# EPFL-VILAB/omnidata

Measured on AMD Instinct MI355X. Metric: images/sec (384x384) DPT-Hybrid surface-normal inference, higher is better.
Workload: dtype bf16; 1 GPU; DPT-Hybrid-384 normal, batch 32/GPU, bf16, 1xMI355X (BASELINE.json configs[1]); batch_per_gpu=32, global_batch=32, parallelism=replicas x1 (no collective in the loop), ranks_seen=1, inflight=1

## Files before the change

include/dptx.h:

```cpp
#ifndef DPTX_H_
#define DPTX_H_

#include <stddef.h>
#include <stdint.h>

#ifdef __cplusplus
extern "C" {
#endif

typedef struct dptx_engine* dptx_handle;

enum {
  DPTX_OK = 0,
  DPTX_E_INVALID = -1,
  DPTX_E_KEY = -2,
  DPTX_E_HIP = -3,
  DPTX_E_NODEVICE = -4,
  DPTX_E_ALLOC = -5
};

enum { DPTX_DTYPE_BF16 = 0, DPTX_DTYPE_FP16 = 1, DPTX_DTYPE_BF16X3 = 2,
       DPTX_DTYPE_FP16X3 = 3, DPTX_DTYPE_MIXED = 4,
       DPTX_DTYPE_FP8 = 5 };
enum { DPTX_GROUP_RESNET = 1,
// ... 165 lines not shown
int dptx_eval_normal_pixels(const float* pred, const float* target, int32_t B, int32_t H, int32_t W, double* ang, void* stream);


int dptx_op_set_planes(int64_t act_plane_elems, int64_t w_plane_elems);

int dptx_op_gemm(int32_t dtype, const void* A, const void* W, const float* bias, const void* R,
                 void* C, int32_t M, int32_t N, int32_t K, int32_t act, int32_t a_fp32,
                 int32_t c_fp32, int32_t r_fp32, void* stream);
int dptx_op_conv(int32_t dtype, const void* X, const void* Wt, const float* bias, const void* R,
                 void* Y, int32_t B, int32_t H, int32_t W, int32_t Cin, int32_t Cout,
                 int32_t ksize, int32_t stride, int32_t pad_t, int32_t pad_l, int32_t Ho,
                 int32_t Wo, int32_t a_relu, int32_t act, void* stream);
int dptx_op_conv_planes(int32_t dtype, const void* X, const void* Wt, const float* bias, const void* R, void* Y, int32_t B,
                        int32_t H, int32_t W, int32_t Cin, int32_t Cout, int32_t ksize, int32_t stride, int32_t pad_t,
                        int32_t pad_l, int32_t Ho, int32_t Wo, int32_t a_relu, int32_t act, int32_t epi2, int32_t c_hi_only,
                        int32_t r1_hi_only, void* stream);
int dptx_op_stem_conv(int32_t dtype, const float* x, const void* Wt, void* y, int32_t B, int32_t H, int32_t W,
                      void* stream);
int dptx_op_attention(int32_t dtype, const void* qkv, void* out, int32_t B, int32_t S,
                      int32_t heads, void* stream);
int dptx_op_layernorm(int32_t dtype, const float* x, const float* gamma, const float* beta,
                      void* y, int32_t M, int32_t C, float eps, void* stream);
int dptx_op_groupnorm(int32_t dtype, const void* X, const float* gamma, const float* beta,
                      const void* R, void* Y, int32_t B, int32_t HW, int32_t C, int32_t relu,
                      float eps, void* scratch_f32, void* stream);
int dptx_op_gn_relu_maxpool(int32_t dtype, const void* X, const float* gamma, const float* beta, void* Y, int32_t B,
                            int32_t H, int32_t W, int32_t C, float eps, void* scratch_f32, void* stream);
int dptx_op_cls_rows(int32_t dtype, const float* cls, const float* pos, float* X, int32_t B, int32_t S, int32_t C, void* X16,
                     float* row_stats, void* X8, float q_scale, void* stream);
int dptx_debug_set_trace(void* dev_buf);
int dptx_debug_arena_fill(dptx_handle h, int32_t byte_value);
int dptx_debug_arena_read(dptx_handle h, void* dst_host, size_t offset, size_t bytes);
int dptx_debug_arena_layout(dptx_handle h, char* dst, size_t capacity);
int dptx_debug_arena_checksums(dptx_handle h, void* out_dev, int32_t capacity, void* stream);
int dptx_debug_set_gemm_flags(int32_t flags);
int dptx_op_conv_fp8(const void* X8, const void* Wt8, const float* bias, const void* R, void* Y, void* Y8, int32_t B,
                     int32_t H, int32_t W, int32_t Cin, int32_t Cout, int32_t ksize, int32_t stride, int32_t pad_t,
                     int32_t pad_l, int32_t Ho, int32_t Wo, int32_t act, int32_t q_relu, float out_scale, void* stream);
int dptx_op_conv_groupnorm(int32_t dtype, const void* X, const void* Wt, void* Yraw, const float* gamma, const float* beta,
                           const void* R, void* Y, int32_t B, int32_t H, int32_t W, int32_t Cin, int32_t Cout,
                           int32_t ksize, int32_t stride, int32_t pad_t, int32_t pad_l, int32_t Ho, int32_t Wo,
                           int32_t relu, float eps, void* scratch_f32, void* stream);
int dptx_op_upsample2x(int32_t dtype, const void* X, void* Y, int32_t B, int32_t H, int32_t W,
                       int32_t C, void* stream);
int dptx_op_gemm_ln(int32_t dtype, const void* A, const void* W, const float* bias, void* C, int32_t M, int32_t N, int32_t K,
                    int32_t act, const float* ln_stats, const float* ln_colsum, int32_t ln_nblk, float ln_eps, void* stream);
int dptx_op_gemm_stream(int32_t dtype, const void* A, const void* W, const float* bias, void* C, float* row_stats, int32_t M,
                        int32_t N, int32_t K, void* stream);
int dptx_op_gemm_stream32(int32_t dtype, const void* A, const void* W, const float* bias, float* X, void* C16, float* row_stats,
                          int32_t M, int32_t N, int32_t K, void* stream);
int dptx_op_head_tail(int32_t dtype, const void* H0, const void* W2, const float* b2, const float* w4,
                      const float* b4, float* y, int32_t B, int32_t Hs, int32_t Ws, int32_t C,
                      int32_t relu_out, void* stream);

#ifdef __cplusplus
}
#endif
#endif
```

omnidata_amd/csrc/head.hip:

```cpp
#include <cstdlib>

#include "common.h"
#include "kernels.h"

namespace dptx {

constexpr int HT_THREADS = 576;
constexpr int HT_PR = 10, HT_PC = 34;
constexpr int HT_W_BYTES = 32 * 9 * 256;
constexpr int HT_P_BYTES = HT_PR * HT_PC * 256;
constexpr int HT_CONST_FLOATS = 32 + 3 * 32 + 4;
constexpr size_t HT_SMEM = HT_W_BYTES + HT_P_BYTES + HT_CONST_FLOATS * 4;

template <int DT>
__device__ __forceinline__ void unpack8(const u32x4_t v, float* f) {
  f[0] = T16<DT>::tof((uint16_t)(v.x & 0xffffu)); f[1] = T16<DT>::tof((uint16_t)(v.x >> 16));
  f[2] = T16<DT>::tof((uint16_t)(v.y & 0xffffu)); f[3] = T16<DT>::tof((uint16_t)(v.y >> 16));
  f[4] = T16<DT>::tof((uint16_t)(v.z & 0xffffu)); f[5] = T16<DT>::tof((uint16_t)(v.z >> 16));
  f[6] = T16<DT>::tof((uint16_t)(v.w & 0xffffu)); f[7] = T16<DT>::tof((uint16_t)(v.w >> 16));
}

template <int DT>
__device__ __forceinline__ void hblend(const u32x4_t s0, const u32x4_t s1, float lx0, float lx1, float (&t)[8]) {
  float a[8], b[8];
  unpack8<DT>(s0, a);
  unpack8<DT>(s1, b);
#pragma unroll
  for (int e = 0; e < 8; ++e) t[e] = __fmaf_rn(lx1, b[e], __fmul_rn(lx0, a[e]));
}
template <int DT, int J>
__device__ __forceinline__ u32x4_t vblend(const float (&T)[6][8], float ly0, float ly1) {
  float o[8];
#pragma unroll
  for (int e = 0; e < 8; ++e) o[e] = __fmaf_rn(ly1, T[J + 1][e], __fmul_rn(ly0, T[J][e]));
  u32x4_t r;
  r.x = T16<DT>::pack2(o[0], o[1]);
  r.y = T16<DT>::pack2(o[2], o[3]);
  r.z = T16<DT>::pack2(o[4], o[5]);
  r.w = T16<DT>::pack2(o[6], o[7]);
  return r;
}

template <int DT>
__global__ __launch_bounds__(HT_THREADS) void head_tail_kernel(const uint16_t* __restrict__ H0, const uint16_t* __restrict__ W2,
                                                               const float* __restrict__ b2, const float* __restrict__ w4,
                                                               const float* __restrict__ b4, void* __restrict__ y, int io, int B,
                                                               int Hs, int Ws, int C, int relu_out, int ntiles) {
  extern __shared__ __attribute__((aligned(16))) char smem[];
  char* Wl = smem;
  char* P = smem + HT_W_BYTES;
  float* cst = (float*)(smem + HT_W_BYTES + HT_P_BYTES);

  const int tid = threadIdx.x, lane = tid & 63, wave = tid >> 6;
  const int lr = lane & 31, lh = lane >> 5;
  const int Ho = 2 * Hs, Wo = 2 * Ws;
  const int tiles_x = Wo / 32, tiles_y = Ho / 8, tpi = tiles_x * tiles_y;
  const float ry = Ho > 1 ? (float)(Hs - 1) / (float)(Ho - 1) : 0.f;
  const float rx = Wo > 1 ? (float)(Ws - 1) / (float)(Wo - 1) : 0.f;

  {
    constexpr int NW = 32 * 9 * 16 / HT_THREADS;
    static_assert(NW * HT_THREADS == 32 * 9 * 16, "weight tensor splits evenly over the block");
    u32x4_t wv[NW];
#pragma unroll
    for (int j = 0; j < NW; ++j) {
      const int i = tid + j * HT_THREADS;
      const int n = i / 144, rem = i - n * 144;
      wv[j] = *(const u32x4_t*)(W2 + n * 1152 + (rem >> 4) * 128 + (rem & 15) * 8);
    }
#pragma unroll
    for (int j = 0; j < NW; ++j) {
      const int i = tid + j * HT_THREADS;
      const int n = i / 144, rem = i - n * 144, tap = rem >> 4, ch = rem & 15;
      *(u32x4_t*)(Wl + n * 2304 + tap * 256 + ((ch ^ (n & 15)) << 4)) = wv[j];
    }
  }
  if (tid < 32) cst[tid] = b2[tid];
  if (tid < 32 * C) cst[32 + tid] = w4[tid];
  if (tid < C) cst[128 + tid] = b4[tid];

  const int per = (ntiles + gridDim.x - 1) / gridDim.x;
  const int t_beg = blockIdx.x * per, t_end = min(t_beg + per, ntiles);

  const int wx = tid >> 4, wch = tid & 15;
  const bool col_thread = wx < HT_PC;

  u32x4_t S[6][2];
  const u32x4_t zero4 = {0u, 0u, 0u, 0u};

  auto fetch = [&](int t) {
    const int b = t / tpi, rem = t - b * tpi, ty = rem / tiles_x, tx = rem - ty * tiles_x;
    const int ox = tx * 32 - 1 + wx;
    const bool vx = col_thread && ox >= 0 && ox < Wo;
    const float sx = rx * (float)(vx ? ox : 0);
    const int x0 = (int)sx, x1 = x0 + (x0 < Ws - 1 ? 1 : 0);
    const int oyb = max(ty * 8 - 1, 0);
    const int ybase = (int)(ry * (float)oyb);
    const uint16_t* img = H0 + (long long)b * Hs * Ws * 128 + wch * 8;
#pragma unroll
    for (int j = 0; j < 6; ++j) {
      const int row = min(ybase + j, Hs - 1);
      S[j][0] = vx ? *(const u32x4_t*)(img + ((long long)row * Ws + x0) * 128) : zero4;
      S[j][1] = vx ? *(const u32x4_t*)(img + ((long long)row * Ws + x1) * 128) : zero4;
    }
  };

  if (t_beg < t_end) fetch(t_beg);
  __syncthreads();

  for (int t = t_beg; t < t_end; ++t) {
    const int b = t / tpi, rem = t - b * tpi, ty = rem / tiles_x, tx = rem - ty * tiles_x;
    const int oy0 = ty * 8, ox0 = tx * 32;

    if (col_thread) {
      const int ox = ox0 - 1 + wx;
      const bool vx = ox >= 0 && ox < Wo;
      const float sx = rx * (float)(vx ? ox : 0);
      const int x0 = (int)sx;
      const float lx1 = sx - (float)x0, lx0 = 1.f - lx1;
      const int ybase = (int)(ry * (float)max(oy0 - 1, 0));
      char* dst = P + wx * 256 + ((wch ^ (wx & 15)) << 4);
      float T[6][8];
#pragma unroll
      for (int j = 0; j < 6; ++j) hblend<DT>(S[j][0], S[j][1], lx0, lx1, T[j]);
      for (int r = 0; r < HT_PR; ++r) {
        const int oy = oy0 - 1 + r;
        u32x4_t o = zero4;
        if (vx && oy >= 0 && oy < Ho) {
          const float sy = ry * (float)oy;
          const int y0 = (int)sy;
          const float ly1 = sy - (float)y0, ly0 = 1.f - ly1;
          switch (y0 - ybase) {
            case 0: o = vblend<DT, 0>(T, ly0, ly1); break;
            case 1: o = vblend<DT, 1>(T, ly0, ly1); break;
            case 2: o = vblend<DT, 2>(T, ly0, ly1); break;
            case 3: o = vblend<DT, 3>(T, ly0, ly1); break;
            default: o = vblend<DT, 4>(T, ly0, ly1); break;
          }
        }
        *(u32x4_t*)(dst + r * (HT_PC * 256)) = o;
      }
    }
    if (t + 1 < t_end) fetch(t + 1);
    __syncthreads();

    if (wave < 8) {
      f32x16_t acc;
#pragma unroll
      for (int r = 0; r < 16; ++r) acc[r] = 0.f;
      const char* wrow = Wl + lr * 2304;
      const int wkey = lr & 15;
      constexpr int NB = 2, NBATCH = 8 / NB * 9;
      u32x4_t wf[2][NB], pf[2][NB];
      auto read_batch = [&](int bi, u32x4_t (&w)[NB], u32x4_t (&q)[NB]) {
        const int tap = bi / (8 / NB), cb0 = (bi % (8 / NB)) * NB;
        const int ky = tap / 3, kx = tap - ky * 3;
        const int xc = lr + kx;
        const char* prow = P + ((wave + ky) * HT_PC + xc) * 256;
        const int pkey = xc & 15;
#pragma unroll
        for (int i = 0; i < NB; ++i) {
          const int chunk = 2 * (cb0 + i) + lh;
          w[i] = *(const u32x4_t*)(wrow + tap * 256 + ((chunk ^ wkey) << 4));
          q[i] = *(const u32x4_t*)(prow + ((chunk ^ pkey) << 4));
        }
      };
      read_batch(0, wf[0], pf[0]);
#pragma unroll
      for (int bi = 0; bi < NBATCH; ++bi) {
        if (bi + 1 < NBATCH) read_batch(bi + 1, wf[(bi + 1) & 1], pf[(bi + 1) & 1]);
        __builtin_amdgcn_sched_barrier(0);
#pragma unroll
        for (int i = 0; i < NB; ++i) acc = T16<DT>::mfma32(wf[bi & 1][i], pf[bi & 1][i], acc);
        __builtin_amdgcn_sched_barrier(0);
      }
      float h[16];
#pragma unroll
      for (int q = 0; q < 4; ++q) {
        const float4 bb = *(const float4*)(cst + 8 * q + 4 * lh);
        h[4 * q + 0] = fmaxf(acc[4 * q + 0] + bb.x, 0.f);
        h[4 * q + 1] = fmaxf(acc[4 * q + 1] + bb.y, 0.f);
        h[4 * q + 2] = fmaxf(acc[4 * q + 2] + bb.z, 0.f);
        h[4 * q + 3] = fmaxf(acc[4 * q + 3] + bb.w, 0.f);
      }
      const int oy = oy0 + wave;
      for (int c = 0; c < C; ++c) {
        float s = 0.f;
#pragma unroll
        for (int q = 0; q < 4; ++q) {
          const float4 ww = *(const float4*)(cst + 32 + c * 32 + 8 * q + 4 * lh);
          s += ww.x * h[4 * q + 0] + ww.y * h[4 * q + 1] + ww.z * h[4 * q + 2] + ww.w * h[4 * q + 3];
        }
        s += __shfl_xor(s, 32);
        s += cst[128 + c];
        if (relu_out) s = fmaxf(s, 0.f);
        if ((c & 1) == lh) io_store(y, (((long long)b * C + c) * Ho + oy) * Wo + ox0 + lr, s, io);
      }
    }
    __syncthreads();
  }
}

constexpr int HX_THREADS = 640;
constexpr int HX_WPL = 9 * 32 * 64;
constexpr int HX_PPL = HT_PR * HT_PC * 64;
constexpr int HX_STAGE = 2 * HX_WPL + 2 * HX_PPL;
constexpr size_t HX_SMEM = 2 * HX_STAGE;
static_assert(HX_SMEM <= 160 * 1024, "one block per CU");

template <int DT>
__device__ __forceinline__ void hblend2(const u32x4_t (&s0)[2], const u32x4_t (&s1)[2], float lx0, float lx1, float (&t)[8]) {
  float a[8], b[8];
  unpack8x<DT, 2>(s0[0], s0[1], a);
  unpack8x<DT, 2>(s1[0], s1[1], b);
#pragma unroll
  for (int e = 0; e < 8; ++e) t[e] = __fmaf_rn(lx1, b[e], __fmul_rn(lx0, a[e]));
}

template <int DT>
__global__ __launch_bounds__(HX_THREADS) void head_tail_x3_kernel(const uint16_t* __restrict__ H0, const uint16_t* __restrict__ W2,
                                                                  const float* __restrict__ b2, const float* __restrict__ w4,
                                                                  const float* __restrict__ b4, void* __restrict__ y, int io, int B,
                                                                  int Hs, int Ws, int C, int relu_out, int ntiles, long long plane,
                                                                  long long wplane) {
#if defined(__HIP_DEVICE_COMPILE__)
  extern __shared__ __attribute__((aligned(16))) char smem[];

  const int tid = threadIdx.x, lane = tid & 63;
  const int wave = __builtin_amdgcn_readfirstlane(tid >> 6);
  const int lr = lane & 31, lh = lane >> 5;
  const int Ho = 2 * Hs, Wo = 2 * Ws;
  const int tiles_x = Wo / 32, tiles_y = Ho / 8, tpi = tiles_x * tiles_y;
  const float ry = Ho > 1 ? (float)(Hs - 1) / (float)(Ho - 1) : 0.f;
  const float rx = Wo > 1 ? (float)(Ws - 1) / (float)(Wo - 1) : 0.f;

  const int per = (ntiles + gridDim.x - 1) / gridDim.x;
  const int t_beg = blockIdx.x * per, t_end = min(t_beg + per, ntiles);
  const int G = (t_end - t_beg) * 4;
  if (G <= 0) return;

  if (wave == 5) {
    const __amdgpu_buffer_rsrc_t rsrcW = __builtin_amdgcn_make_buffer_rsrc(const_cast<uint16_t*>(W2), 0, (int)((wplane + 32 * 1152) * 2), 0x00020000);
#pragma unroll 1
    for (int g = 0; g < G; ++g) {
      const int quarter = g & 3;
      char* Wl = smem + (g & 1) * HX_STAGE;
#pragma unroll 6
      for (int q = 0; q < 36; ++q) {
        const int pl = q / 18, r = 16 * (q % 18) + (lane >> 2);
        const int tap = r >> 5, n = r & 31;
        const int sch = (lane & 3) ^ ((n >> 2) & 3);
        const unsigned off = (unsigned)(((long long)pl * wplane + n * 1152 + tap * 128 + quarter * 32 + sch * 8) * 2);
        __builtin_amdgcn_raw_ptr_buffer_load_lds(rsrcW, (__attribute__((address_space(3))) void*)(Wl + q * 1024), 16, off, 0, 0, 0);
// ... 108 lines not shown
      }
    };
    read_ks(0, 0, wf[0], pf[0]);
#pragma unroll
    for (int ks = 0; ks < 18; ++ks) {
      if (ks + 1 < 18) read_ks((ks + 1) >> 1, (ks + 1) & 1, wf[(ks + 1) & 1], pf[(ks + 1) & 1]);
      __builtin_amdgcn_sched_barrier(0);
      acc[0] = T16<DT>::mfma32(wf[ks & 1][0], pf[ks & 1][0][1], acc[0]);
      acc[1] = T16<DT>::mfma32(wf[ks & 1][0], pf[ks & 1][1][1], acc[1]);
      acc[0] = T16<DT>::mfma32(wf[ks & 1][1], pf[ks & 1][0][0], acc[0]);
      acc[1] = T16<DT>::mfma32(wf[ks & 1][1], pf[ks & 1][1][0], acc[1]);
      acc[0] = T16<DT>::mfma32(wf[ks & 1][0], pf[ks & 1][0][0], acc[0]);
      acc[1] = T16<DT>::mfma32(wf[ks & 1][0], pf[ks & 1][1][0], acc[1]);
      __builtin_amdgcn_sched_barrier(0);
    }
    if (quarter == 3) {
      const int b = t / tpi, rem = t - b * tpi, ty = rem / tiles_x, tx = rem - ty * tiles_x;
      const int oy0 = ty * 8, ox0 = tx * 32;
#pragma unroll
      for (int i = 0; i < 2; ++i) {
        float h[16];
#pragma unroll
        for (int q = 0; q < 4; ++q) {
          const float4 bb = *(const float4*)(b2 + 8 * q + 4 * lh);
          h[4 * q + 0] = fmaxf(acc[i][4 * q + 0] + bb.x, 0.f);
          h[4 * q + 1] = fmaxf(acc[i][4 * q + 1] + bb.y, 0.f);
          h[4 * q + 2] = fmaxf(acc[i][4 * q + 2] + bb.z, 0.f);
          h[4 * q + 3] = fmaxf(acc[i][4 * q + 3] + bb.w, 0.f);
        }
        const int oy = oy0 + 2 * mw + i;
        for (int c = 0; c < C; ++c) {
          float sacc = 0.f;
#pragma unroll
          for (int q = 0; q < 4; ++q) {
            const float4 ww = *(const float4*)(w4 + c * 32 + 8 * q + 4 * lh);
            sacc += ww.x * h[4 * q + 0] + ww.y * h[4 * q + 1] + ww.z * h[4 * q + 2] + ww.w * h[4 * q + 3];
          }
          sacc += __shfl_xor(sacc, 32);
          sacc += b4[c];
          if (relu_out) sacc = fmaxf(sacc, 0.f);
          if ((c & 1) == lh) io_store(y, (((long long)b * C + c) * Ho + oy) * Wo + ox0 + lr, sacc, io);
        }
      }
    }
    if (g + 1 < G) {
      asm volatile("s_waitcnt lgkmcnt(0)" ::: "memory");
      asm volatile("s_barrier" ::: "memory");
    }
  }
#endif
}

hipError_t launch_head_tail(int mode, const void* H0, const void* W2, const float* b2, const float* w4, const float* b4,
                            void* y, int io, int B, int Hs, int Ws, int C, int relu_out, hipStream_t stream, Planes pl) {
  if (C < 1 || C > 3 || (2 * Hs) % 8 != 0 || (2 * Ws) % 32 != 0) return hipErrorInvalidValue;
  const int ntiles = B * ((2 * Hs) / 8) * ((2 * Ws) / 32);
  static int cus = 0;
  if (cus == 0) {
    int dev = 0;
    hipDeviceProp_t prop;
    if (hipGetDevice(&dev) == hipSuccess && hipGetDeviceProperties(&prop, dev) == hipSuccess) cus = prop.multiProcessorCount;
    if (cus <= 0) cus = 256;
  }
  const int grid = ntiles < cus ? ntiles : cus;
  if (mode_is_x3(mode)) {
    if (mode != MODE_FP16X3 || pl.act == 0 || pl.w == 0 || (pl.w + 32 * 1152) * 2 >= (1ll << 31)) return hipErrorInvalidValue;
    auto k = head_tail_x3_kernel<DT_FP16>;
    ensure_dyn_smem((const void*)k, HX_SMEM);
    const int grid2 = grid;
    hipLaunchKernelGGL(k, dim3(grid2), dim3(HX_THREADS), HX_SMEM, stream, (const uint16_t*)H0, (const uint16_t*)W2, b2, w4, b4, y, io, B,
                       Hs, Ws, C, relu_out, ntiles, pl.act, pl.w);
    return hipGetLastError();
  }
  if (mode == MODE_BF16) {
    auto k = head_tail_kernel<DT_BF16>;
    ensure_dyn_smem((const void*)k, HT_SMEM);
    hipLaunchKernelGGL(k, dim3(grid), dim3(HT_THREADS), HT_SMEM, stream, (const uint16_t*)H0, (const uint16_t*)W2, b2, w4, b4, y, io, B,
                       Hs, Ws, C, relu_out, ntiles);
  } else {
    auto k = head_tail_kernel<DT_FP16>;
    ensure_dyn_smem((const void*)k, HT_SMEM);
    hipLaunchKernelGGL(k, dim3(grid), dim3(HT_THREADS), HT_SMEM, stream, (const uint16_t*)H0, (const uint16_t*)W2, b2, w4, b4, y, io, B,
                       Hs, Ws, C, relu_out, ntiles);
  }
  return hipGetLastError();
}

}
```

omnidata_amd/csrc/kernels.h:

```cpp
#pragma once
#include <hip/hip_runtime.h>
#include <stdint.h>

#include "common.h"

namespace dptx {

void ensure_dyn_smem(const void* kernel, size_t bytes);

struct GemmParams {
  const void* A;
  const void* W;
  void* C;
  const float* bias;
  const void* R1;
  const void* R2;
  int M, N, K;
  int ldw;
  int a_rpi, Wout, Hin, Win, Cin, a_pix_stride;
  long long a_img_stride, a_off;
  long long a_bytes;
  int ksz, stride, pad_t, pad_l;
  int c_rpi, c_img_rows, c_row_off, ldc;
  int r2_bcast;
// ... 25 lines not shown
  long long* trace;
  int debug_flags;
  float a_rpi_rcp, wout_rcp;
};

void gemm_params_dense(GemmParams& p, int M, int N, int K);
void gemm_params_conv(GemmParams& p, int B, int Hin, int Win, int Cin, int Cout, int ksz, int stride, int pad_t, int pad_l,
                      int Hout, int Wout, int a_elem_bytes);
hipError_t launch_gemm(int dtype, const GemmParams& p, hipStream_t stream);
void gemm_set_trace(long long* dev_buf);
void gemm_set_debug_flags(int flags);
bool conv1x1_stream_eligible(int mode, const GemmParams& p);
bool conv1x1_stream_adopted(const GemmParams& p);
hipError_t launch_conv1x1_stream(int mode, const GemmParams& p, hipStream_t stream);
void gemm_set_cu_share(float share);

hipError_t launch_attention(int mode, const void* qkv, void* out, int B, int S, int heads, Planes pl, hipStream_t stream);

hipError_t launch_layernorm(int mode, const float* x, const float* gamma, const float* beta, void* y,
                            int M, int C, float eps, Planes pl, hipStream_t stream);

struct GnParams {
  const void* X; void* Y;
  const float* gamma; const float* beta;
  float* partial;
  const void* R;
  const float* r_gamma; const float* r_beta; const float* r_partial;
  int B, HW, C, relu;
  float eps;
  int nrec;
};
int gn_chunks(int HW, int C);
hipError_t launch_gn_stats(int mode, const void* X, float* partial, int B, int HW, int C, Planes pl, hipStream_t stream);
hipError_t launch_gn_apply(int mode, const GnParams& p, Planes pl, hipStream_t stream);
hipError_t launch_gn_relu_maxpool(int mode, const void* X, void* Y, const float* gamma, const float* beta,
                                  const float* partial, int B, int H, int W, int C, float eps, Planes pl, hipStream_t stream);

hipError_t launch_stem_conv(int mode, const void* x, int io, const void* Wt, void* y, int B, int H, int W, Planes pl,
                            hipStream_t stream);

hipError_t launch_upsample2x(int mode, const void* X, void* Y, int B, int H, int W, int C, Planes pl, hipStream_t stream,
                             void* Y8 = nullptr, float q_scale = 1.0f, bool out_hi_only = false);
hipError_t launch_amax(int mode, const void* X, size_t n, int relu, unsigned* amax_bits, hipStream_t stream);

hipError_t launch_nonfinite_scan(int mode, const void* X, size_t n, unsigned* flag, hipStream_t stream);

hipError_t launch_checksum(const void* p, size_t bytes, unsigned long long* out, hipStream_t stream);
hipError_t launch_spin(long long ticks_100mhz, hipStream_t stream);

hipError_t launch_head_out(int mode, const void* X, const float* w, const float* b, void* y, int io, int B, int HW,
                           int Cout, int relu, Planes pl, hipStream_t stream);

hipError_t launch_head_tail(int mode, const void* H0, const void* W2, const float* b2, const float* w4, const float* b4,
                            void* y, int io, int B, int Hs, int Ws, int C, int relu_out, hipStream_t stream, Planes pl = Planes{0, 0});
hipError_t launch_pos_resize(const float* src, float* dst, int g_old, int gh, int gw, int C, hipStream_t stream);
hipError_t launch_cls_rows(int mode, const float* cls, const float* pos, float* X, int B, int S, int C, void* X16, float* stats,
                           hipStream_t stream, void* X8 = nullptr, float q_scale = 1.0f);

hipError_t launch_readout_cls(int mode, const float* x, long long x_stride, const void* W, int ldw, int w_off,
                              const float* bias, float* out, int B, int N, int K, Planes pl, hipStream_t stream, int x16 = 0);
hipError_t launch_cast_f32(int mode, const float* src, void* dst, size_t n, Planes pl, hipStream_t stream);

hipError_t launch_patchify16(int mode, const void* x, int io, void* P, int B, int H, int W, Planes pl, hipStream_t stream);
hipError_t launch_depth_to_space(int mode, const void* G, void* Y, int B, int h, int w, int k, int C, Planes pl, hipStream_t stream);

hipError_t launch_to_f32(int mode, const void* src, float* dst, size_t n, Planes pl, hipStream_t stream);

}
```

omnidata_amd/csrc/ops.hip:

```cpp
#include <hip/hip_runtime.h>

#include "../../include/dptx.h"
#include "kernels.h"

using namespace dptx;

extern "C" {

static int rc(hipError_t r) { return r == hipSuccess ? DPTX_OK : DPTX_E_HIP; }

static Planes g_op_planes{0, 0};
int dptx_op_set_planes(int64_t act_plane_elems, int64_t w_plane_elems) {
  g_op_planes.act = act_plane_elems;
  g_op_planes.w = w_plane_elems;
  return DPTX_OK;
}

int dptx_op_gemm(int32_t dtype, const void* A, const void* W, const float* bias, const void* R, void* C, int32_t M, int32_t N,
                 int32_t K, int32_t act, int32_t a_fp32, int32_t c_fp32, int32_t r_fp32, void* stream) {
  GemmParams p;
  gemm_params_dense(p, M, N, K);
  p.A = A; p.W = W; p.C = C; p.bias = bias; p.R1 = R; p.act = act; p.a_fp32 = a_fp32; p.c_fp32 = c_fp32; p.r1_fp32 = r_fp32;
  p.planes = g_op_planes;
  return rc(launch_gemm(dtype, p, (hipStream_t)stream));
}

int dptx_op_gemm_ln(int32_t dtype, const void* A, const void* W, const float* bias, void* C, int32_t M, int32_t N, int32_t K,
                    int32_t act, const float* ln_stats, const float* ln_colsum, int32_t ln_nblk, float ln_eps, void* stream) {
  GemmParams p;
  gemm_params_dense(p, M, N, K);
  p.A = A; p.W = W; p.C = C; p.bias = bias; p.act = act; p.planes = g_op_planes;
  p.ln_stats = ln_stats; p.ln_colsum = ln_colsum; p.ln_nblk = ln_nblk; p.ln_eps = ln_eps; p.ln_inv_dim = 1.0f / (float)K;
  return rc(launch_gemm(dtype, p, (hipStream_t)stream));
}

int dptx_op_gemm_stream(int32_t dtype, const void* A, const void* W, const float* bias, void* C, float* row_stats, int32_t M,
                        int32_t N, int32_t K, void* stream) {
  GemmParams p;
  gemm_params_dense(p, M, N, K);
  p.A = A; p.W = W; p.C = C; p.R1 = C; p.bias = bias; p.planes = g_op_planes;
  p.row_stats = row_stats; p.stats_nblk = 8;
  return rc(launch_gemm(dtype, p, (hipStream_t)stream));
}

int dptx_op_gemm_stream32(int32_t dtype, const void* A, const void* W, const float* bias, float* X, void* C16, float* row_stats,
                          int32_t M, int32_t N, int32_t K, void* stream) {
  GemmParams p;
  gemm_params_dense(p, M, N, K);
  p.A = A; p.W = W; p.C = X; p.c_fp32 = 1; p.R1 = X; p.r1_fp32 = 1; p.C16 = C16; p.bias = bias; p.planes = g_op_planes;
  p.row_stats = row_stats; p.stats_nblk = 8;
  return rc(launch_gemm(dtype, p, (hipStream_t)stream));
}

int dptx_op_head_tail(int32_t dtype, const void* H0, const void* W2, const float* b2, const float* w4, const float* b4, float* y,
                      int32_t B, int32_t Hs, int32_t Ws, int32_t C, int32_t relu_out, void* stream) {
  return rc(launch_head_tail(dtype, H0, W2, b2, w4, b4, y, DPTX_IO_FP32, B, Hs, Ws, C, relu_out, (hipStream_t)stream, g_op_planes));
}

int dptx_op_conv(int32_t dtype, const void* X, const void* Wt, const float* bias, const void* R, void* Y, int32_t B, int32_t H,
                 int32_t W, int32_t Cin, int32_t Cout, int32_t ksize, int32_t stride, int32_t pad_t, int32_t pad_l, int32_t Ho,
                 int32_t Wo, int32_t a_relu, int32_t act, void* stream) {
  GemmParams p;
  gemm_params_conv(p, B, H, W, Cin, Cout, ksize, stride, pad_t, pad_l, Ho, Wo, 2);
  p.A = X; p.W = Wt; p.C = Y; p.bias = bias; p.R1 = R; p.act = act; p.a_relu = a_relu; p.planes = g_op_planes;
  return rc(launch_gemm(dtype, p, (hipStream_t)stream));
}

int dptx_op_conv_planes(int32_t dtype, const void* X, const void* Wt, const float* bias, const void* R, void* Y, int32_t B, int32_t H,
                        int32_t W, int32_t Cin, int32_t Cout, int32_t ksize, int32_t stride, int32_t pad_t, int32_t pad_l, int32_t Ho,
                        int32_t Wo, int32_t a_relu, int32_t act, int32_t epi2, int32_t c_hi_only, int32_t r1_hi_only, void* stream) {
  GemmParams p;
  gemm_params_conv(p, B, H, W, Cin, Cout, ksize, stride, pad_t, pad_l, Ho, Wo, 2);
  p.A = X; p.W = Wt; p.C = Y; p.bias = bias; p.R1 = R; p.act = act; p.a_relu = a_relu; p.planes = g_op_planes;
  p.epi2 = epi2 & 1; p.a_hi_only = (epi2 >> 1) & 1; p.c_hi_only = c_hi_only; p.r1_hi_only = r1_hi_only;
  return rc(launch_gemm(dtype, p, (hipStream_t)stream));
}

int dptx_op_stem_conv(int32_t dtype, const float* x, const void* Wt, void* y, int32_t B, int32_t H, int32_t W, void* stream) {
  return rc(launch_stem_conv(dtype, x, DPTX_IO_FP32, Wt, y, B, H, W, g_op_planes, (hipStream_t)stream));
}

int dptx_op_attention(int32_t dtype, const void* qkv, void* out, int32_t B, int32_t S, int32_t heads, void* stream) {
  return rc(launch_attention(dtype, qkv, out, B, S, heads, g_op_planes, (hipStream_t)stream));
}

int dptx_op_layernorm(int32_t dtype, const float* x, const float* gamma, const float* beta, void* y, int32_t M, int32_t C,
                      float eps, void* stream) {
  return rc(launch_layernorm(dtype, x, gamma, beta, y, M, C, eps, g_op_planes, (hipStream_t)stream));
}

int dptx_op_groupnorm(int32_t dtype, const void* X, const float* gamma, const float* beta, const void* R, void* Y, int32_t B,
                      int32_t HW, int32_t C, int32_t relu, float eps, void* scratch_f32, void* stream) {
  if (scratch_f32 == nullptr) return DPTX_E_INVALID;
  hipError_t r = launch_gn_stats(dtype, X, (float*)scratch_f32, B, HW, C, g_op_planes, (hipStream_t)stream);
  if (r != hipSuccess) return DPTX_E_HIP;
  GnParams g{};
  g.X = X; g.Y = Y; g.gamma = gamma; g.beta = beta; g.partial = (float*)scratch_f32; g.R = R;
  g.B = B; g.HW = HW; g.C = C; g.relu = relu; g.eps = eps;
  return rc(launch_gn_apply(dtype, g, g_op_planes, (hipStream_t)stream));
}

int dptx_op_gn_relu_maxpool(int32_t dtype, const void* X, const float* gamma, const float* beta, void* Y, int32_t B, int32_t H,
                            int32_t W, int32_t C, float eps, void* scratch_f32, void* stream) {
  if (scratch_f32 == nullptr) return DPTX_E_INVALID;
  hipError_t r = launch_gn_stats(dtype, X, (float*)scratch_f32, B, H * W, C, g_op_planes, (hipStream_t)stream);
  if (r != hipSuccess) return DPTX_E_HIP;
  return rc(launch_gn_relu_maxpool(dtype, X, Y, gamma, beta, (const float*)scratch_f32, B, H, W, C, eps, g_op_planes, (hipStream_t)stream));
}

// ... 47 lines not shown
```

omnidata_amd/engine.py:

```python
from __future__ import annotations

import ctypes as C
import os
from typing import Dict, Optional, Tuple

import numpy as np
import torch

_HERE = os.path.dirname(os.path.abspath(__file__))
LIB_PATH = os.environ.get("DPTX_LIB") or os.path.join(_HERE, "libdptx.so")

DTYPES = {"bf16": 0, "fp16": 1, "bf16x3": 2, "fp16x3": 3, "mixed": 4, "fp8": 5}
TWO_PLANE_DTYPES = frozenset(("bf16x3", "fp16x3", "mixed", "fp8"))
GROUPS = {"resnet": 1, "embed": 2, "vit": 4, "reassemble": 8, "rn": 16, "fusion": 32, "head": 64, "all": 127}
FLAGS = {"no_ln_fold": 1, "group_policy": 2, "fp32_stream": 4, "no_range_check": 8, "fp8_all": 16, "fp8_vit": 32}


def groups_mask(names) -> int:
    if isinstance(names, int):
        return names
    if isinstance(names, str):
        names = [n for n in names.replace(",", "+").split("+") if n]
    mask = 0
    for n in names:
# ... 50 lines not shown
    ("dptx_postprocess_normal_u8", C.c_int, [_vp, _vp, _vp]),
    ("dptx_postprocess_depth", C.c_int, [_vp, _vp, _vp]),
    ("dptx_resample_coeffs", C.c_int, [_i32, _i32, C.POINTER(C.c_int32), C.POINTER(C.c_int32), _i32, C.POINTER(C.c_int32)]),
    ("dptx_refocus_workspace_bytes", C.c_int, [_i32, _i32, _i32, _i32, _i32, _i64p]),
    ("dptx_refocus_quantiles", C.c_int, [_vp, _i32, _i32, _i32, _i32, _vp, _vp, C.c_int64, _vp]),
    ("dptx_refocus", C.c_int, [_vp, _vp, _i32, _i32, _i32, _i32, _i32, _vp, _vp, _vp, _vp, _vp, _vp, C.c_int64, _vp]),
    ("dptx_midas_workspace_bytes", C.c_int, [_i32, _i32, _i32, _i32, _i64p]),
    ("dptx_midas_loss", C.c_int, [_vp, _vp, _vp, _i32, _i32, _i32, _i32, _i32, _i32, C.c_float, _vp, _vp, _vp, C.c_int64, _vp]),
    ("dptx_midas_loss_backward", C.c_int, [_vp, _vp, _vp, _i32, _i32, _i32, _i32, _i32, _i32, C.c_float, _vp, _vp, _vp, _vp]),
    ("dptx_midas_stats", C.c_int, [_vp, _vp, _vp, _i32, _i32, _i32, _i32, _vp, _vp, _vp, _vp, C.c_int64, _vp]),
    ("dptx_vnl_workspace_bytes", C.c_int, [_i32, _i32, _i32, _i32, _i64p]),
    ("dptx_vnl_prepare", C.c_int, [_vp, _vp, _vp, _i32, _i32, _i32, _vp, _vp, C.c_int64, _vp]),
    ("dptx_vnl_loss", C.c_int, [_vp, _vp, _i32, _i32, _i32, C.c_float, C.c_float, C.c_float, _vp, _vp, _vp, _i32, _i32, _vp, _vp,
                                _vp, C.c_int64, _vp]),
    ("dptx_vnl_loss_backward", C.c_int, [_vp, _vp, _i32, _i32, _i32, C.c_float, C.c_float, _vp, _vp, _vp, _i32, _vp, _vp, _vp, _vp,
                                         _vp, _vp]),
    ("dptx_vnl_triples", C.c_int, [_vp, _vp, _i32, _i32, _i32, C.c_float, C.c_float, C.c_float, _vp, _vp, _vp, _i32, _vp, _vp, _vp,
                                   _vp]),
    ("dptx_normal_workspace_bytes", C.c_int, [_i32, _i32, _i32, _i64p]),
    ("dptx_normal_loss", C.c_int, [_vp, _vp, _vp, _i32, _i32, _i32, _i32, C.c_float, _vp, _vp, _vp, C.c_int64, _vp]),
    ("dptx_normal_loss_backward", C.c_int, [_vp, _vp, _vp, _i32, _i32, _i32, _i32, C.c_float, _vp, _vp, _vp, _vp]),
    ("dptx_normal_pixels", C.c_int, [_vp, _vp, _vp, _i32, _i32, _i32, _i32, _vp, _vp, _vp]),
    ("dptx_masked_workspace_bytes", C.c_int, [C.c_int64, _i64p]),
    ("dptx_masked_loss", C.c_int, [_vp, _vp, _vp, C.c_int64, _i32, _vp, _vp, _vp, C.c_int64, _vp]),
    ("dptx_masked_loss_backward", C.c_int, [_vp, _vp, _vp, C.c_int64, _i32, _vp, _vp, _vp, _vp]),
    ("dptx_valid_mask", C.c_int, [_vp, _i32, _i32, _i32, _i32, _vp, _vp]),
    ("dptx_eval_workspace_bytes", C.c_int, [_i32, _i32, _i32, _i64p]),
    ("dptx_eval_normal", C.c_int, [_vp, _vp, _vp, _i32, _i32, _i32, _i32, _vp, _vp, C.c_int64, _vp]),
    ("dptx_eval_depth", C.c_int, [_vp, _vp, _vp, _i32, _i32, _i32, _i32, _vp, _vp, C.c_int64, _vp]),
    ("dptx_eval_normal_pixels", C.c_int, [_vp, _vp, _i32, _i32, _i32, _vp, _vp]),
    ("dptx_op_set_planes", C.c_int, [C.c_int64, C.c_int64]),
    ("dptx_op_gemm", C.c_int, [_i32, _vp, _vp, _vp, _vp, _vp, _i32, _i32, _i32, _i32, _i32, _i32, _i32, _vp]),
    ("dptx_op_conv", C.c_int, [_i32, _vp, _vp, _vp, _vp, _vp] + [_i32] * 13 + [_vp]),
    ("dptx_op_conv_planes", C.c_int, [_i32, _vp, _vp, _vp, _vp, _vp] + [_i32] * 16 + [_vp]),
    ("dptx_op_stem_conv", C.c_int, [_i32, _vp, _vp, _vp, _i32, _i32, _i32, _vp]),
    ("dptx_op_attention", C.c_int, [_i32, _vp, _vp, _i32, _i32, _i32, _vp]),
    ("dptx_op_layernorm", C.c_int, [_i32, _vp, _vp, _vp, _vp, _i32, _i32, C.c_float, _vp]),
    ("dptx_op_groupnorm", C.c_int, [_i32, _vp, _vp, _vp, _vp, _vp, _i32, _i32, _i32, _i32, C.c_float, _vp, _vp]),
    ("dptx_op_gn_relu_maxpool", C.c_int, [_i32, _vp, _vp, _vp, _vp, _i32, _i32, _i32, _i32, C.c_float, _vp, _vp]),
    ("dptx_op_cls_rows", C.c_int, [_i32, _vp, _vp, _vp, _i32, _i32, _i32, _vp, _vp, _vp, C.c_float, _vp]),
    ("dptx_debug_set_trace", C.c_int, [_vp]),
    ("dptx_debug_set_gemm_flags", C.c_int, [C.c_int32]),
    ("dptx_debug_arena_fill", C.c_int, [_vp, _i32]),
    ("dptx_debug_arena_read", C.c_int, [_vp, _vp, _sz, _sz]),
    ("dptx_debug_arena_layout", C.c_int, [_vp, C.c_char_p, _sz]),
    ("dptx_debug_arena_checksums", C.c_int, [_vp, _vp, _i32, _vp]),
    ("dptx_op_conv_fp8", C.c_int, [_vp, _vp, _vp, _vp, _vp, _vp] + [_i32] * 13 + [C.c_float, _vp]),
    ("dptx_op_conv_groupnorm", C.c_int, [_i32, _vp, _vp, _vp, _vp, _vp, _vp, _vp] + [_i32] * 12 + [C.c_float, _vp, _vp]),
    ("dptx_op_upsample2x", C.c_int, [_i32, _vp, _vp, _i32, _i32, _i32, _i32, _vp]),
    ("dptx_op_gemm_ln", C.c_int, [_i32, _vp, _vp, _vp, _vp, _i32, _i32, _i32, _i32, _vp, _vp, _i32, C.c_float, _vp]),
    ("dptx_op_gemm_stream", C.c_int, [_i32, _vp, _vp, _vp, _vp, _vp, _i32, _i32, _i32, _vp]),
    ("dptx_op_gemm_stream32", C.c_int, [_i32, _vp, _vp, _vp, _vp, _vp, _vp, _i32, _i32, _i32, _vp]),
    ("dptx_op_head_tail", C.c_int, [_i32, _vp, _vp, _vp, _vp, _vp, _vp, _i32, _i32, _i32, _i32, _i32, _vp]),
]

_lib = None


def _embedded_hash(path: str) -> str:
    import re
    try:
        with open(path, "rb") as f:
            data = f.read()
    except OSError:
        return ""
    m = re.search(rb"dptx [0-9.]+ \(gfx950[^)]*\) src=([0-9a-f]{16})", data)
    return m.group(1).decode() if m else ""


def load_library() -> C.CDLL:
    global _lib
    if _lib is None:
        check = not os.environ.get("DPTX_LIB") and not os.environ.get("DPTX_SKIP_HASH_CHECK")
        want = ""
        if check:
            from .build import build, source_hash
            want = source_hash(os.environ.get("DPTX_CXXFLAGS", "").split())
            have = _embedded_hash(LIB_PATH) if os.path.exists(LIB_PATH) else ""
            if have != want:
                hipcc = os.environ.get("HIPCC", "/opt/rocm/bin/hipcc")
                if not os.path.exists(hipcc):
                    raise RuntimeError(f"{LIB_PATH} is {'stale (built from sources ' + have + ')' if have else 'missing'}; the tree "
                                       f"has {want} and {hipcc} is not available: run `python -m omnidata_amd.build` on a "
                                       "machine with ROCm. There is no CPU fallback.")
                build()
        if not os.path.exists(LIB_PATH):
            raise RuntimeError(f"{LIB_PATH} not found: run `python -m omnidata_amd.build` "
                               "(or __graft_entry__.build()). There is no CPU fallback.")
        lib = C.CDLL(LIB_PATH)
        for name, res, args in ABI:
            fn = getattr(lib, name)
            fn.restype = res
            fn.argtypes = args
        if check:
            built = lib.dptx_version().decode().rsplit("src=", 1)[-1]
            if built != want:
                raise RuntimeError(f"{LIB_PATH} is stale: built from sources {built}, the tree has {want}. "
                                   "Run `python -m omnidata_amd.build --force`.")
        _lib = lib
    return _lib


def _ptr(t) -> int:
    return 0 if t is None else t.data_ptr()


# ... 305 lines not shown
```

Before: 2701 images/s.

## Warp-specialize head tail kernel into builder and MFMA waves over vertical strips

The head tail kernel now uses 13 waves per block: 9 builder waves upsample input rows into a 10-row ring buffer in LDS, and 4 MFMA waves compute the 3x3 conv plus 1x1 output for 4 rows per step. Blocks walk vertical 32-column strips in 4-row steps, so the halo rows built for one step are reused by the next instead of rebuilding 10 rows for each 8-row tile. The goal is to overlap the bilinear-upsample build with the conv and to cut redundant halo upsampling. The change adds more barriers per output row, a modulo-indexed ring, and a debug entry point to cap the grid size.

```diff
diff --git a/include/dptx.h b/include/dptx.h
--- a/include/dptx.h
+++ b/include/dptx.h
@@ -241,6 +241,9 @@
 int dptx_op_head_tail(int32_t dtype, const void* H0, const void* W2, const float* b2, const float* w4,
                       const float* b4, float* y, int32_t B, int32_t Hs, int32_t Ws, int32_t C,
                       int32_t relu_out, void* stream);
+int dptx_op_head_tail_blocks(int32_t dtype, const void* H0, const void* W2, const float* b2, const float* w4,
+                             const float* b4, float* y, int32_t B, int32_t Hs, int32_t Ws, int32_t C,
+                             int32_t relu_out, int32_t max_blocks, void* stream);
 
 #ifdef __cplusplus
 }
diff --git a/omnidata_amd/csrc/head.hip b/omnidata_amd/csrc/head.hip
--- a/omnidata_amd/csrc/head.hip
+++ b/omnidata_amd/csrc/head.hip
@@ -5,12 +5,17 @@
 
 namespace dptx {
 
-constexpr int HT_THREADS = 576;
+constexpr int HT_MULT_WAVES = 4, HT_BUILD_WAVES = 9;
+constexpr int HT_THREADS = (HT_MULT_WAVES + HT_BUILD_WAVES) * 64;
 constexpr int HT_PR = 10, HT_PC = 34;
+constexpr int HT_NB = 2;
+constexpr int HT_ITEMS = HT_PC * 16;
+constexpr int HT_ROW_BYTES = HT_PC * 256;
 constexpr int HT_W_BYTES = 32 * 9 * 256;
-constexpr int HT_P_BYTES = HT_PR * HT_PC * 256;
+constexpr int HT_P_BYTES = HT_PR * HT_ROW_BYTES;
 constexpr int HT_CONST_FLOATS = 32 + 3 * 32 + 4;
 constexpr size_t HT_SMEM = HT_W_BYTES + HT_P_BYTES + HT_CONST_FLOATS * 4;
+static_assert(HT_ITEMS <= HT_BUILD_WAVES * 64, "one item per builder lane");
 
 template <int DT>
 __device__ __forceinline__ void unpack8(const u32x4_t v, float* f) {
@@ -28,8 +33,9 @@
 #pragma unroll
   for (int e = 0; e < 8; ++e) t[e] = __fmaf_rn(lx1, b[e], __fmul_rn(lx0, a[e]));
 }
-template <int DT, int J>
-__device__ __forceinline__ u32x4_t vblend(const float (&T)[6][8], float ly0, float ly1) {
+template <int DT, int J, int NR>
+__device__ __forceinline__ u32x4_t vblend(const float (&T)[NR][8], float ly0, float ly1) {
+  static_assert(J + 1 < NR, "two neighbouring source rows");
   float o[8];
 #pragma unroll
   for (int e = 0; e < 8; ++e) o[e] = __fmaf_rn(ly1, T[J + 1][e], __fmul_rn(ly0, T[J][e]));
@@ -41,128 +47,164 @@
   return r;
 }
 
+__device__ __forceinline__ void src_index(float ratio, int dst, int& i0, float& l0, float& l1) {
+  const float fd = (float)dst;
+  i0 = (int)__fmul_rn(ratio, fd);
+  l1 = __fmaf_rn(ratio, fd, -(float)i0);
+  l0 = __fsub_rn(1.f, l1);
+}
+
+__device__ __forceinline__ void ht_barrier() {
+  asm volatile("s_waitcnt lgkmcnt(0)\n\ts_barrier" ::: "memory");
+}
+
 template <int DT>
 __global__ __launch_bounds__(HT_THREADS) void head_tail_kernel(const uint16_t* __restrict__ H0, const uint16_t* __restrict__ W2,
                                                                const float* __restrict__ b2, const float* __restrict__ w4,
                                                                const float* __restrict__ b4, void* __restrict__ y, int io, int B,
-                                                               int Hs, int Ws, int C, int relu_out, int ntiles) {
+                                                               int Hs, int Ws, int C, int relu_out, int nsteps) {
   extern __shared__ __attribute__((aligned(16))) char smem[];
   char* Wl = smem;
   char* P = smem + HT_W_BYTES;
   float* cst = (float*)(smem + HT_W_BYTES + HT_P_BYTES);
 
-  const int tid = threadIdx.x, lane = tid & 63, wave = tid >> 6;
+  const int tid = threadIdx.x, lane = tid & 63;
+  const int wave = __builtin_amdgcn_readfirstlane(tid >> 6);
   const int lr = lane & 31, lh = lane >> 5;
   const int Ho = 2 * Hs, Wo = 2 * Ws;
-  const int tiles_x = Wo / 32, tiles_y = Ho / 8, tpi = tiles_x * tiles_y;
+  const int strips_x = Wo / 32, spy = Ho / 4;
   const float ry = Ho > 1 ? (float)(Hs - 1) / (float)(Ho - 1) : 0.f;
   const float rx = Wo > 1 ? (float)(Ws - 1) / (float)(Wo - 1) : 0.f;
 
+  const int per = (nsteps + gridDim.x - 1) / gridDim.x;
+  const int s_beg = blockIdx.x * per, s_end = min(s_beg + per, nsteps);
+  if (s_beg >= s_end) return;
+
   {
-    constexpr int NW = 32 * 9 * 16 / HT_THREADS;
-    static_assert(NW * HT_THREADS == 32 * 9 * 16, "weight tensor splits evenly over the block");
+    constexpr int NV = 32 * 9 * 16, NW = (NV + HT_THREADS - 1) / HT_THREADS;
     u32x4_t wv[NW];
 #pragma unroll
     for (int j = 0; j < NW; ++j) {
       const int i = tid + j * HT_THREADS;
       const int n = i / 144, rem = i - n * 144;
-      wv[j] = *(const u32x4_t*)(W2 + n * 1152 + (rem >> 4) * 128 + (rem & 15) * 8);
+      if (i < NV) wv[j] = *(const u32x4_t*)(W2 + n * 1152 + (rem >> 4) * 128 + (rem & 15) * 8);
     }
 #pragma unroll
     for (int j = 0; j < NW; ++j) {
       const int i = tid + j * HT_THREADS;
       const int n = i / 144, rem = i - n * 144, tap = rem >> 4, ch = rem & 15;
-      *(u32x4_t*)(Wl + n * 2304 + tap * 256 + ((ch ^ (n & 15)) << 4)) = wv[j];
+      if (i < NV) *(u32x4_t*)(Wl + n * 2304 + tap * 256 + ((ch ^ (n & 15)) << 4)) = wv[j];
     }
   }
   if (tid < 32) cst[tid] = b2[tid];
   if (tid < 32 * C) cst[32 + tid] = w4[tid];
   if (tid < C) cst[128 + tid] = b4[tid];
 
-  const int per = (ntiles + gridDim.x - 1) / gridDim.x;
-  const int t_beg = blockIdx.x * per, t_end = min(t_beg + per, ntiles);
-
-  const int wx = tid >> 4, wch = tid & 15;
-  const bool col_thread = wx < HT_PC;
-
-  u32x4_t S[6][2];
+  const int item = tid - HT_MULT_WAVES * 64;
+  const bool has_item = item >= 0 && item < HT_ITEMS;
+  const int wx = item >> 4, wch = item & 15;
+
+  u32x4_t S[4][2];
   const u32x4_t zero4 = {0u, 0u, 0u, 0u};
 
-  auto fetch = [&](int t) {
-    const int b = t / tpi, rem = t - b * tpi, ty = rem / tiles_x, tx = rem - ty * tiles_x;
-    const int ox = tx * 32 - 1 + wx;
-    const bool vx = col_thread && ox >= 0 && ox < Wo;
-    const float sx = rx * (float)(vx ? ox : 0);
-    const int x0 = (int)sx, x1 = x0 + (x0 < Ws - 1 ? 1 : 0);
-    const int oyb = max(ty * 8 - 1, 0);
-    const int ybase = (int)(ry * (float)oyb);
+  auto fetch4 = [&](int b, int ox0, int row0) __attribute__((always_inline)) {
+    const int ox = ox0 - 1 + wx;
+    const bool vx = ox >= 0 && ox < Wo;
+    const int x0 = (int)__fmul_rn(rx, (float)(vx ? ox : 0)), x1 = x0 + (x0 < Ws - 1 ? 1 : 0);
+    const int ybase = (int)__fmul_rn(ry, (float)max(row0, 0));
     const uint16_t* img = H0 + (long long)b * Hs * Ws * 128 + wch * 8;
 #pragma unroll
-    for (int j = 0; j < 6; ++j) {
-      const int row = min(ybase + j, Hs - 1);
-      S[j][0] = vx ? *(const u32x4_t*)(img + ((long long)row * Ws + x0) * 128) : zero4;
-      S[j][1] = vx ? *(const u32x4_t*)(img + ((long long)row * Ws + x1) * 128) : zero4;
+    for (int q = 0; q < 4; ++q) {
+      const int row = min(ybase + q, Hs - 1);
+      S[q][0] = vx ? *(const u32x4_t*)(img + ((long long)row * Ws + x0) * 128) : zero4;
+      S[q][1] = vx ? *(const u32x4_t*)(img + ((long long)row * Ws + x1) * 128) : zero4;
     }
   };
-
-  if (t_beg < t_end) fetch(t_beg);
-  __syncthreads();
-
-  for (int t = t_beg; t < t_end; ++t) {
-    const int b = t / tpi, rem = t - b * tpi, ty = rem / tiles_x, tx = rem - ty * tiles_x;
-    const int oy0 = ty * 8, ox0 = tx * 32;
-
-    if (col_thread) {
-      const int ox = ox0 - 1 + wx;
-      const bool vx = ox >= 0 && ox < Wo;
-      const float sx = rx * (float)(vx ? ox : 0);
-      const int x0 = (int)sx;
-      const float lx1 = sx - (float)x0, lx0 = 1.f - lx1;
-      const int ybase = (int)(ry * (float)max(oy0 - 1, 0));
-      char* dst = P + wx * 256 + ((wch ^ (wx & 15)) << 4);
-      float T[6][8];
-#pragma unroll
-      for (int j = 0; j < 6; ++j) hblend<DT>(S[j][0], S[j][1], lx0, lx1, T[j]);
-      for (int r = 0; r < HT_PR; ++r) {
-        const int oy = oy0 - 1 + r;
+  auto build4 = [&](int ox0, int row0, int nrows) __attribute__((always_inline)) {
+    const int ox = ox0 - 1 + wx;
+    const bool vx = ox >= 0 && ox < Wo;
+    int x0;
+    float lx0, lx1;
+    src_index(rx, vx ? ox : 0, x0, lx0, lx1);
+    const int ybase = (int)__fmul_rn(ry, (float)max(row0, 0));
+    char* dst = P + wx * 256 + ((wch ^ (wx & 15)) << 4);
+    float T[4][8];
+#pragma unroll
+    for (int q = 0; q < 4; ++q) hblend<DT>(S[q][0], S[q][1], lx0, lx1, T[q]);
+#pragma unroll
+    for (int r = 0; r < 4; ++r) {
+      if (r < nrows) {
+        const int oy = row0 + r;
         u32x4_t o = zero4;
         if (vx && oy >= 0 && oy < Ho) {
-          const float sy = ry * (float)oy;
-          const int y0 = (int)sy;
-          const float ly1 = sy - (float)y0, ly0 = 1.f - ly1;
+          int y0;
+          float ly0, ly1;
+          src_index(ry, oy, y0, ly0, ly1);
           switch (y0 - ybase) {
             case 0: o = vblend<DT, 0>(T, ly0, ly1); break;
             case 1: o = vblend<DT, 1>(T, ly0, ly1); break;
-            case 2: o = vblend<DT, 2>(T, ly0, ly1); break;
-            case 3: o = vblend<DT, 3>(T, ly0, ly1); break;
-            default: o = vblend<DT, 4>(T, ly0, ly1); break;
+            default: o = vblend<DT, 2>(T, ly0, ly1); break;
           }
         }
-        *(u32x4_t*)(dst + r * (HT_PC * 256)) = o;
-      }
-    }
-    if (t + 1 < t_end) fetch(t + 1);
-    __syncthreads();
-
-    if (wave < 8) {
+        *(u32x4_t*)(dst + ((oy + 1) % HT_PR) * HT_ROW_BYTES) = o;
+      }
+    }
+  };
+
+  auto walk = [&](auto&& prime, auto&& step) __attribute__((always_inline)) {
+    for (int s = s_beg; s < s_end; ++s) {
+      const int strip = s / spy, j = s - strip * spy;
+      const int b = strip / strips_x, ox0 = (strip - b * strips_x) * 32;
+      const int seg_end = min(s_end, (strip + 1) * spy);
+      if (s == s_beg || j == 0) {
+        prime(s, seg_end, b, ox0, j);
+        ht_barrier();
+      }
+      step(s, seg_end, b, ox0, j);
+      ht_barrier();
+    }
+  };
+
+  if (wave >= HT_MULT_WAVES) {
+    walk(
+        [&](int s, int seg_end, int b, int ox0, int j) __attribute__((always_inline)) {
+          if (!has_item) return;
+          fetch4(b, ox0, 4 * j - 1);
+          build4(ox0, 4 * j - 1, 4);
+          fetch4(b, ox0, 4 * j + 3);
+          build4(ox0, 4 * j + 3, 2);
+          if (s + 1 < seg_end) fetch4(b, ox0, 4 * j + 5);
+        },
+        [&](int s, int seg_end, int b, int ox0, int j) __attribute__((always_inline)) {
+          if (!has_item || s + 1 >= seg_end) return;
+          build4(ox0, 4 * j + 5, 4);
+          if (s + 2 < seg_end) fetch4(b, ox0, 4 * j + 9);
+        });
+    return;
+  }
+  walk([](int, int, int, int, int) {},
+       [&](int, int, int b, int ox0, int j) __attribute__((always_inline)) {
       f32x16_t acc;
 #pragma unroll
       for (int r = 0; r < 16; ++r) acc[r] = 0.f;
       const char* wrow = Wl + lr * 2304;
       const int wkey = lr & 15;
-      constexpr int NB = 2, NBATCH = 8 / NB * 9;
+      int prow[3];
+#pragma unroll
+      for (int ky = 0; ky < 3; ++ky) prow[ky] = ((4 * j + wave + ky) % HT_PR) * HT_ROW_BYTES;
+      constexpr int NB = HT_NB, NBATCH = 8 / NB * 9;
       u32x4_t wf[2][NB], pf[2][NB];
       auto read_batch = [&](int bi, u32x4_t (&w)[NB], u32x4_t (&q)[NB]) {
         const int tap = bi / (8 / NB), cb0 = (bi % (8 / NB)) * NB;
         const int ky = tap / 3, kx = tap - ky * 3;
         const int xc = lr + kx;
-        const char* prow = P + ((wave + ky) * HT_PC + xc) * 256;
+        const char* pr = P + prow[ky] + xc * 256;
         const int pkey = xc & 15;
 #pragma unroll
         for (int i = 0; i < NB; ++i) {
           const int chunk = 2 * (cb0 + i) + lh;
           w[i] = *(const u32x4_t*)(wrow + tap * 256 + ((chunk ^ wkey) << 4));
-          q[i] = *(const u32x4_t*)(prow + ((chunk ^ pkey) << 4));
+          q[i] = *(const u32x4_t*)(pr + ((chunk ^ pkey) << 4));
         }
       };
       read_batch(0, wf[0], pf[0]);
@@ -183,22 +225,20 @@
         h[4 * q + 2] = fmaxf(acc[4 * q + 2] + bb.z, 0.f);
         h[4 * q + 3] = fmaxf(acc[4 * q + 3] + bb.w, 0.f);
       }
-      const int oy = oy0 + wave;
+      const int oy = 4 * j + wave;
       for (int c = 0; c < C; ++c) {
-        float s = 0.f;
+        float sum = 0.f;
 #pragma unroll
         for (int q = 0; q < 4; ++q) {
           const float4 ww = *(const float4*)(cst + 32 + c * 32 + 8 * q + 4 * lh);
-          s += ww.x * h[4 * q + 0] + ww.y * h[4 * q + 1] + ww.z * h[4 * q + 2] + ww.w * h[4 * q + 3];
-        }
-        s += __shfl_xor(s, 32);
-        s += cst[128 + c];
-        if (relu_out) s = fmaxf(s, 0.f);
-        if ((c & 1) == lh) io_store(y, (((long long)b * C + c) * Ho + oy) * Wo + ox0 + lr, s, io);
-      }
-    }
-    __syncthreads();
-  }
+          sum += ww.x * h[4 * q + 0] + ww.y * h[4 * q + 1] + ww.z * h[4 * q + 2] + ww.w * h[4 * q + 3];
+        }
+        sum += __shfl_xor(sum, 32);
+        sum += cst[128 + c];
+        if (relu_out) sum = fmaxf(sum, 0.f);
+        if ((c & 1) == lh) io_store(y, (((long long)b * C + c) * Ho + oy) * Wo + ox0 + lr, sum, io);
+      }
+       });
 }
 
 constexpr int HX_THREADS = 640;
@@ -413,8 +453,8 @@
 }
 
 hipError_t launch_head_tail(int mode, const void* H0, const void* W2, const float* b2, const float* w4, const float* b4,
-                            void* y, int io, int B, int Hs, int Ws, int C, int relu_out, hipStream_t stream, Planes pl) {
-  if (C < 1 || C > 3 || (2 * Hs) % 8 != 0 || (2 * Ws) % 32 != 0) return hipErrorInvalidValue;
+                            void* y, int io, int B, int Hs, int Ws, int C, int relu_out, hipStream_t stream, Planes pl, int max_blocks) {
+  if (C < 1 || C > 3 || (2 * Hs) % 8 != 0 || (2 * Ws) % 32 != 0 || max_blocks < 0) return hipErrorInvalidValue;
   const int ntiles = B * ((2 * Hs) / 8) * ((2 * Ws) / 32);
   static int cus = 0;
   if (cus == 0) {
@@ -423,26 +463,28 @@
     if (hipGetDevice(&dev) == hipSuccess && hipGetDeviceProperties(&prop, dev) == hipSuccess) cus = prop.multiProcessorCount;
     if (cus <= 0) cus = 256;
   }
-  const int grid = ntiles < cus ? ntiles : cus;
+  const int blocks = max_blocks > 0 ? max_blocks : cus;
   if (mode_is_x3(mode)) {
     if (mode != MODE_FP16X3 || pl.act == 0 || pl.w == 0 || (pl.w + 32 * 1152) * 2 >= (1ll << 31)) return hipErrorInvalidValue;
     auto k = head_tail_x3_kernel<DT_FP16>;
     ensure_dyn_smem((const void*)k, HX_SMEM);
-    const int grid2 = grid;
+    const int grid2 = ntiles < blocks ? ntiles : blocks;
     hipLaunchKernelGGL(k, dim3(grid2), dim3(HX_THREADS), HX_SMEM, stream, (const uint16_t*)H0, (const uint16_t*)W2, b2, w4, b4, y, io, B,
                        Hs, Ws, C, relu_out, ntiles, pl.act, pl.w);
     return hipGetLastError();
   }
+  const int nsteps = 2 * ntiles;
+  const int grid = nsteps < blocks ? nsteps : blocks;
   if (mode == MODE_BF16) {
     auto k = head_tail_kernel<DT_BF16>;
     ensure_dyn_smem((const void*)k, HT_SMEM);
     hipLaunchKernelGGL(k, dim3(grid), dim3(HT_THREADS), HT_SMEM, stream, (const uint16_t*)H0, (const uint16_t*)W2, b2, w4, b4, y, io, B,
-                       Hs, Ws, C, relu_out, ntiles);
+                       Hs, Ws, C, relu_out, nsteps);
   } else {
     auto k = head_tail_kernel<DT_FP16>;
     ensure_dyn_smem((const void*)k, HT_SMEM);
     hipLaunchKernelGGL(k, dim3(grid), dim3(HT_THREADS), HT_SMEM, stream, (const uint16_t*)H0, (const uint16_t*)W2, b2, w4, b4, y, io, B,
-                       Hs, Ws, C, relu_out, ntiles);
+                       Hs, Ws, C, relu_out, nsteps);
   }
   return hipGetLastError();
 }
diff --git a/omnidata_amd/csrc/kernels.h b/omnidata_amd/csrc/kernels.h
--- a/omnidata_amd/csrc/kernels.h
+++ b/omnidata_amd/csrc/kernels.h
@@ -101,7 +101,8 @@
                            int Cout, int relu, Planes pl, hipStream_t stream);
 
 hipError_t launch_head_tail(int mode, const void* H0, const void* W2, const float* b2, const float* w4, const float* b4,
-                            void* y, int io, int B, int Hs, int Ws, int C, int relu_out, hipStream_t stream, Planes pl = Planes{0, 0});
+                            void* y, int io, int B, int Hs, int Ws, int C, int relu_out, hipStream_t stream, Planes pl = Planes{0, 0},
+                            int max_blocks = 0);
 hipError_t launch_pos_resize(const float* src, float* dst, int g_old, int gh, int gw, int C, hipStream_t stream);
 hipError_t launch_cls_rows(int mode, const float* cls, const float* pos, float* X, int B, int S, int C, void* X16, float* stats,
                            hipStream_t stream, void* X8 = nullptr, float q_scale = 1.0f);
diff --git a/omnidata_amd/csrc/ops.hip b/omnidata_amd/csrc/ops.hip
--- a/omnidata_amd/csrc/ops.hip
+++ b/omnidata_amd/csrc/ops.hip
@@ -55,6 +55,13 @@
 int dptx_op_head_tail(int32_t dtype, const void* H0, const void* W2, const float* b2, const float* w4, const float* b4, float* y,
                       int32_t B, int32_t Hs, int32_t Ws, int32_t C, int32_t relu_out, void* stream) {
   return rc(launch_head_tail(dtype, H0, W2, b2, w4, b4, y, DPTX_IO_FP32, B, Hs, Ws, C, relu_out, (hipStream_t)stream, g_op_planes));
+}
+
+int dptx_op_head_tail_blocks(int32_t dtype, const void* H0, const void* W2, const float* b2, const float* w4, const float* b4,
+                             float* y, int32_t B, int32_t Hs, int32_t Ws, int32_t C, int32_t relu_out, int32_t max_blocks,
+                             void* stream) {
+  return rc(launch_head_tail(dtype, H0, W2, b2, w4, b4, y, DPTX_IO_FP32, B, Hs, Ws, C, relu_out, (hipStream_t)stream, g_op_planes,
+                             max_blocks));
 }
 
 int dptx_op_conv(int32_t dtype, const void* X, const void* Wt, const float* bias, const void* R, void* Y, int32_t B, int32_t H,
diff --git a/omnidata_amd/engine.py b/omnidata_amd/engine.py
--- a/omnidata_amd/engine.py
+++ b/omnidata_amd/engine.py
@@ -126,6 +126,7 @@
     ("dptx_op_gemm_stream", C.c_int, [_i32, _vp, _vp, _vp, _vp, _vp, _i32, _i32, _i32, _vp]),
     ("dptx_op_gemm_stream32", C.c_int, [_i32, _vp, _vp, _vp, _vp, _vp, _vp, _i32, _i32, _i32, _vp]),
     ("dptx_op_head_tail", C.c_int, [_i32, _vp, _vp, _vp, _vp, _vp, _vp, _i32, _i32, _i32, _i32, _i32, _vp]),
+    ("dptx_op_head_tail_blocks", C.c_int, [_i32, _vp, _vp, _vp, _vp, _vp, _vp, _i32, _i32, _i32, _i32, _i32, _i32, _vp]),
 ]
 
 _lib = None
```

New measurement: 2714 images/s (median of 6 runs). Within noise of the previous version (+0.5%).
